# JohannesErnst/WeaSAL

Measured on AMD Instinct MI355X. Metric: points/sec fwd+bwd KPFCNN on DALES spheres; achieved HBM GB/s on KPConv gather, higher is better.
Workload: dtype f32; 1 GPU; DALES_PseudoLabel KP-FCNN, in_radius=10m, 50k pts/sphere, batch=8, fp32, step = GPU pyramid + fwd + loss + bwd + SGD; contrast_loss term included (trainer_PseudoLabel.py:204-208); pyramid of the next batch overlapped on a second stream; parallelism=dp1, dist_world_size=1, allreduce_bytes=0

## Files before the change

### weasal_amd/csrc/blocks.hip

```cpp
#include <vector>

#include "ws_common.h"

extern "C" int ws_block_gates = 1;
extern "C" int ws_block_gather_residual = 1;
extern "C" int64_t ws_block_group_rows = (int64_t)1 << 62;
extern "C" int ws_block_fused_infer = 1;
extern "C" int ws_block_pool_order = 1;
extern "C" int ws_block_packed_k4 = 1;

namespace {

struct Arena {
    char* base;
    int64_t cap, off;
    Arena(void* b, int64_t c) : base((char*)b), cap(c), off(0) {}
    template <typename T> T* take(int64_t count)
    {
        off = (off + 255) & ~(int64_t)255;
        T* p = base ? reinterpret_cast<T*>(base + off) : nullptr;
        off += count * (int64_t)sizeof(T);
        return p;
    }
    bool fits() const { return off <= cap; }
// ... 32 lines not shown
               int act, float slope, float* y, float* tr, void* tmp, int64_t tmp_bytes, hipStream_t st)
{
    if (l.in_place())
        return ws_gemm_xb_epilogue_strided(x, m, l.k, ldx, l.w, 1, l.ldw, l.n, bias, residual, ldr, act, slope, y, l.n, tmp, tmp_bytes, st);
    transpose_small_kernel<<<(unsigned)ws_ceil_div((int64_t)l.k * l.n, 256), 256, 0, st>>>(l.w, l.n, l.k, l.ldw, tr);
    return ws_gemm_xb_epilogue_strided(x, m, l.k, ldx, tr, l.n, 1, l.n, bias, residual, ldr, act, slope, y, l.n, tmp, tmp_bytes, st);
}

#define WS_TRY(call)            \
    do {                        \
        int rc__ = (call);      \
        if (rc__) return rc__;  \
    } while (0)

inline bool grouped_rows(int64_t rows) { return ws_block_group_rows > 0 && rows > 0 && rows < ws_block_group_rows; }

inline ws_xb_problem xb_problem(const float* x, int64_t m, int k, int64_t ldx, const float* b, int64_t brs, int64_t bcs, int n,
                                const float* bias, const float* residual, int64_t ldr, int act, float slope, const float* gate_y,
                                int64_t ldg, float gate_slope, float* y, int64_t ldy, void* scratch, int64_t scratch_bytes)
{
    ws_xb_problem q{};
    q.x = x; q.m = m; q.k = k; q.ldx = ldx; q.b = b; q.b_row_stride = brs; q.b_col_stride = bcs; q.n = n;
    q.bias = bias; q.residual = residual; q.ldr = ldr; q.act = act; q.slope = slope;
    q.gate_y = gate_y; q.ldg = ldg; q.gate_slope = gate_slope;
    q.y = y; q.ldy = ldy; q.scratch = scratch; q.scratch_bytes = scratch_bytes;
    return q;
}

struct Leaves {
    bool on;
// ... 52 lines not shown
{
    int64_t t = ws_gemm_xb_scratch_bytes(d->nq, d->k * d->conv_in, d->conv_out);
    if (d->w1) t = max3(t, ws_gemm_xb_scratch_bytes(d->ns, d->in_dim, d->conv_in), 0);
    if (d->w2) t = max3(t, ws_gemm_xb_scratch_bytes(d->nq, d->conv_out, d->out_dim), d->ws ? ws_gemm_xb_scratch_bytes(d->nq, d->in_dim, d->out_dim) : 0);
    return t;
}

int kpblock_fwd(const ws_kpblock* d, Arena& ar, hipStream_t st, bool run)
{
    const int64_t nq = d->nq, ns = d->ns;
    const Lin l1{d->w1, d->conv_in, d->in_dim, d->in_dim}, l2{d->w2, d->out_dim, d->conv_out, d->conv_out},
        lsc{d->ws, d->out_dim, d->in_dim, d->in_dim};
    float* tr1 = d->w1 ? ar.take<float>(l1.tr_floats()) : nullptr;
    float* tr2 = d->w2 ? ar.take<float>(l2.tr_floats()) : nullptr;
    float* trs = d->ws ? ar.take<float>(lsc.tr_floats()) : nullptr;
    float* sc = (d->w2 && d->ws) ? ar.take<float>(nq * d->out_dim) : nullptr;
    const int64_t tmp_bytes = kpblock_tmp_fwd(d);
    void* tmp = ar.take<char>(tmp_bytes > 16 ? tmp_bytes : 16);
    const bool pair_in = grouped_rows(nq) && d->w1 && d->w2 && d->ws && !d->strided && l1.in_place() && lsc.in_place();
    const int64_t sc_bytes = pair_in ? ws_gemm_xb_scratch_bytes(nq, d->in_dim, d->out_dim) : 0;
    void* tmp_sc = pair_in ? (void*)ar.take<char>(sc_bytes > 16 ? sc_bytes : 16) : nullptr;
    if (!run) return WS_OK;
    if (nq == 0) return WS_OK;
    const float* x1 = d->feat;
    if (pair_in) {
        const ws_xb_problem q[2] = {
            xb_problem(d->feat, ns, l1.k, d->in_dim, l1.w, 1, l1.ldw, l1.n, d->b1, nullptr, 0, 1, d->slope, nullptr, 0, 0.0f, d->x1, l1.n,
                       tmp, tmp_bytes),
            xb_problem(d->feat, nq, lsc.k, d->in_dim, lsc.w, 1, lsc.ldw, lsc.n, d->bs, nullptr, 0, 0, 0.0f, nullptr, 0, 0.0f, sc, lsc.n,
                       tmp_sc, sc_bytes)};
        WS_TRY(ws_priv_gemm_xb_group(q, 2, st));
        x1 = d->x1;
    } else if (d->w1) {
        WS_TRY(linear_fwd(l1, d->feat, ns, d->in_dim, d->b1, nullptr, 0, 1, d->slope, d->x1, tr1, tmp, tmp_bytes, st));
        x1 = d->x1;
    }
    TimerRec rec{};
    if (d->timed) {
        WS_HIP(hipEventCreate(&rec.a));
        WS_HIP(hipEventCreate(&rec.b));
        rec.nq = nq; rec.h = d->h; rec.ci = d->conv_in;
        WS_HIP(hipEventRecord(rec.a, st));
    }
    float* x2 = d->w2 ? d->x2 : d->out;
    const bool one_launch = d->infer && d->k == 15 && d->conv_in == 32 && d->conv_out == 32 && !d->rows_sorted && ((uintptr_t)x1 & 15u) == 0 &&
// ... 5 lines not shown
    } else {
        WS_REQUIRE(d->wf, "wf buffer missing");
        WS_TRY(ws_kpconv_gather_fwd_ex(d->q_pts, nq, d->s_pts, ns, d->inds, d->h, x1, d->conv_in, d->kernel_points, d->k, nullptr,
                                       nullptr, d->extent, WS_INFLUENCE_LINEAR, WS_AGGREGATION_SUM, d->order_q, d->wf, nullptr, 0,
                                       d->rows_sorted, st));
        if (d->timed) WS_HIP(hipEventRecord(rec.b, st));
        WS_TRY(ws_gemm_xb_epilogue_strided(d->wf, nq, d->k * d->conv_in, (int64_t)d->k * d->conv_in, d->wk, d->conv_out, 1, d->conv_out,
                                           d->bk, nullptr, 0, 1, d->slope, x2, d->conv_out, tmp, tmp_bytes, st));
    }
    if (d->timed) {
        WS_HIP(hipEventCreate(&rec.c));
        WS_HIP(hipEventRecord(rec.c, st));
        timer_recs().push_back(rec);
    }
    if (!d->w2) return WS_OK;
    const float* sc_in = d->feat;
    if (d->strided) {
        if (arg_bytes(d))
            WS_TRY(ws_priv_max_pool_fwd_u8(d->feat, ns, d->in_dim, d->inds, nq, d->h, d->pooled, reinterpret_cast<uint8_t*>(d->arg),
                                           ws_block_pool_order ? d->order_q : nullptr, st));
        else
            WS_TRY(ws_max_pool_fwd(d->feat, ns, d->in_dim, d->inds, nq, d->h, d->pooled, d->arg, st));
        sc_in = d->pooled;
    }
    const float* res = sc_in;
    int64_t ldr = d->in_dim;
    if (d->ws) {
        if (!pair_in) WS_TRY(linear_fwd(lsc, sc_in, nq, d->in_dim, d->bs, nullptr, 0, 0, 0.0f, sc, trs, tmp, tmp_bytes, st));
        res = sc;
        ldr = d->out_dim;
    }
    return linear_fwd(l2, x2, nq, d->conv_out, d->b2, res, ldr, 1, d->slope, d->out, tr2, tmp, tmp_bytes, st);
}

int kpblock_bwd(const ws_kpblock* d, Arena& ar, hipStream_t st, bool run)
{
    const int64_t nq = d->nq, ns = d->ns;
    const int kc = d->k * d->conv_in;
    const bool need_dx1 = d->dfeat != nullptr || d->w1 != nullptr;
    const bool want_sc = d->w2 && d->dfeat;
    float* dz = d->w2 ? ar.take<float>(nq * d->out_dim) : nullptr;
    float* g2 = ar.take<float>(nq * d->conv_out);
    float* dwf = need_dx1 ? ar.take<float>(nq * (int64_t)kc) : nullptr;
    float* dx1 = (need_dx1 && d->w1) ? ar.take<float>(ns * d->conv_in) : nullptr;
    float* dscin = (want_sc && d->ws) ? ar.take<float>(nq * d->in_dim) : nullptr;
    float* dfsc = (want_sc && d->strided) ? ar.take<float>(ns * d->in_dim) : nullptr;
    const Lin lk{d->wk, kc, d->conv_out, d->conv_out};
    float* trk = need_dx1 ? ar.take<float>(lk.tr_floats()) : nullptr;
    int64_t tmp_bytes = max3(ws_act_bwd_colsum_scratch_bytes(nq, d->out_dim > d->conv_out ? d->out_dim : d->conv_out),
                             ws_act_bwd_colsum_scratch_bytes(ns, d->conv_in), ws_gemm_xty_scratch_bytes(nq, kc, d->conv_out));
    if (d->w2) tmp_bytes = max3(tmp_bytes, ws_gemm_xty_scratch_bytes(nq, d->out_dim, d->conv_out),
                                d->ws ? ws_gemm_xty_scratch_bytes(nq, d->out_dim, d->in_dim) : 0);
    if (d->w1) tmp_bytes = max3(tmp_bytes, ws_gemm_xty_scratch_bytes(ns, d->conv_in, d->in_dim), 0);
    tmp_bytes = max3(tmp_bytes, ws_gemm_xb_scratch_bytes(nq, d->conv_out, kc), ws_gemm_xb_scratch_bytes(nq, d->out_dim, d->conv_out));
    tmp_bytes = max3(tmp_bytes, ws_gemm_xb_scratch_bytes(nq, d->out_dim, d->in_dim), ws_gemm_xb_scratch_bytes(ns, d->conv_in, d->in_dim));
    void* tmp = ar.take<char>(tmp_bytes > 16 ? tmp_bytes : 16);
    const bool grp = grouped_rows(nq > ns ? nq : ns) && nq > 0 && ns > 0;
    const int64_t b_dwk = ws_gemm_xty_scratch_bytes(nq, kc, d->conv_out);
    const int64_t b_dw2 = d->w2 ? ws_gemm_xty_scratch_bytes(nq, d->out_dim, d->conv_out) : 0;
    const int64_t b_dws = (d->w2 && d->ws) ? ws_gemm_xty_scratch_bytes(nq, d->out_dim, d->in_dim) : 0;
    const int64_t b_dw1 = d->w1 ? ws_gemm_xty_scratch_bytes(ns, d->conv_in, d->in_dim) : 0;
    const int64_t b_g2 = d->w2 ? ws_gemm_xb_scratch_bytes(nq, d->out_dim, d->conv_out) : 0;
    auto own = [&](int64_t bytes) -> void* { return grp ? (void*)ar.take<char>(bytes > 16 ? bytes : 16) : tmp; };
    void* t_dwk = own(b_dwk);
    void* t_dw2 = d->w2 ? own(b_dw2) : tmp;
    void* t_dws = (d->w2 && d->ws) ? own(b_dws) : tmp;
    void* t_dw1 = d->w1 ? own(b_dw1) : tmp;
    void* t_g2 = d->w2 ? own(b_g2) : tmp;
    if (!run) return WS_OK;
    WS_REQUIRE(d->dout && d->dwk, "NULL gradient buffer");
// ... 20 lines not shown
    const float* yconv = d->out;
    WS_REQUIRE(!(d->gate_dfeat && d->dfeat_add && !(d->strided && want_sc)),
               "gate_dfeat with dfeat_add needs the strided shortcut (the sum has to be complete before the gate)");
    if (d->w2) {
        if (d->dout_pregated) {
            if (d->db2) WS_TRY(ws_act_bwd_colsum(d->dout, nq, d->out_dim, d->out_dim, nullptr, 0, 0.0f, nullptr, 0, d->db2, tmp, st));
            dz = const_cast<float*>(d->dout);
        } else
        WS_TRY(ws_act_bwd_colsum(d->dout, nq, d->out_dim, d->out_dim, d->out, d->out_dim, d->slope, dz, d->out_dim, d->db2, tmp, st));
        WS_TRY(leaves.add(dz, nq, d->out_dim, d->out_dim, d->x2, d->conv_out, d->conv_out, d->dw2, 0, t_dw2, b_dw2));
        if (d->ws) {
            const float* sc_in = d->strided ? d->pooled : d->feat;
            WS_TRY(leaves.add(dz, nq, d->out_dim, d->out_dim, sc_in, d->in_dim, d->in_dim, d->dws, 0, t_dws, b_dws));
        }
        gated2 = !d->dbk && ws_block_gates;
        const bool pair_dz = grp && want_sc && d->ws;
        if (pair_dz) {
            const ws_xb_problem q[2] = {
                xb_problem(dz, nq, d->out_dim, d->out_dim, d->ws, d->in_dim, 1, d->in_dim, nullptr, nullptr, 0, 0, 0.0f, nullptr, 0, 0.0f,
                           dscin, d->in_dim, tmp, tmp_bytes),
                xb_problem(dz, nq, d->out_dim, d->out_dim, d->w2, d->conv_out, 1, d->conv_out, nullptr, nullptr, 0, 0, 0.0f,
                           gated2 ? d->x2 : nullptr, d->conv_out, d->slope, g2, d->conv_out, t_g2, b_g2)};
            WS_TRY(ws_priv_gemm_xb_group(q, 2, st));
        }
        if (want_sc) {
            const float* dsc = dz;
            if (d->ws) {
                if (!pair_dz)
                    WS_TRY(ws_gemm_xb_epilogue_strided(dz, nq, d->out_dim, d->out_dim, d->ws, d->in_dim, 1, d->in_dim, nullptr, nullptr, 0,
                                                       0, 0.0f, dscin, d->in_dim, tmp, tmp_bytes, st));
                dsc = dscin;
            }
            if (d->strided) {
                WS_REQUIRE(d->t_offsets && d->t_pairs, "strided block backward needs the transposed table");
                if (arg_bytes(d))
                {
                    WS_TRY(ws_priv_max_pool_bwd_u8(dsc, reinterpret_cast<const uint8_t*>(d->arg), nq, d->h, d->in_dim, d->t_offsets,
                                                   d->t_pairs, ns, dfsc, ws_block_pool_order ? d->order_s : nullptr, d->dfeat_add, st));
                    added = d->dfeat_add != nullptr;
                }
// ... 34 lines not shown
        WS_REQUIRE(d->key_last && d->grid_overflow && nq == ns, "grid backward needs key_last / overflow and a self-query layer");
        WS_TRY(ws_kpconv_gather_bwd_x_grid_gated(d->s_pts, ns, d->grid_blob, d->grid_nb, d->grid_cells, d->key_last, d->grid_radius, dwf,
                                                 d->conv_in, d->kernel_points, d->k, nullptr, nullptr, d->extent, WS_INFLUENCE_LINEAR,
                                                 WS_AGGREGATION_SUM, d->order_s, gate1, d->slope, d->inds, d->h, dx1_out,
                                                 d->grid_overflow, st));
    } else {
        WS_REQUIRE(d->t_offsets && d->t_pairs, "KPConv backward needs the search grid or the transposed table");
        WS_TRY((ws_block_packed_k4 ? ws_kpconv_gather_bwd_x_packed : ws_kpconv_gather_bwd_x_gated)(
            d->q_pts, nq, d->s_pts, ns, d->inds, d->h, d->t_offsets, d->t_pairs, dwf, d->conv_in, d->kernel_points, d->k, nullptr, nullptr,
            d->extent, WS_INFLUENCE_LINEAR, WS_AGGREGATION_SUM, d->order_s, gate1, d->slope, dx1_out, st));
    }
    if (d->w1) {
        if (!gate1)
            WS_TRY(ws_act_bwd_colsum(dx1, ns, d->conv_in, d->conv_in, d->x1, d->conv_in, d->slope, dx1, d->conv_in, d->db1, tmp, st));
        WS_TRY(leaves.add(dx1, ns, d->conv_in, d->conv_in, d->feat, d->in_dim, d->in_dim, d->dw1, 0, t_dw1, b_dw1));
        if (d->dfeat)
            WS_TRY(ws_gemm_xb_gated_strided(dx1, ns, d->conv_in, d->conv_in, d->w1, d->in_dim, 1, d->in_dim, nullptr, sc_res, d->in_dim,
                                            0, 0.0f, d->gate_dfeat ? d->feat : nullptr, d->in_dim, d->slope, nullptr, 0, 0.0f, d->dfeat,
                                            d->in_dim, tmp, tmp_bytes, st));
    } else if (d->dfeat && sc_res) {
        WS_REQUIRE(!d->gate_dfeat, "gate_dfeat: a block without unary1 has no shortcut to add after the gate");
        const int64_t n4 = ns * d->in_dim / 4;
        add_rows_kernel<<<ws_grid(n4, 256), 256, 0, st>>>(d->dfeat, sc_res, n4);
        WS_LAUNCH_CHECK();
    }
    if (d->dfeat && d->dfeat_add && !added) {
        WS_REQUIRE(d->in_dim % 4 == 0, "dfeat_add needs in_dim %% 4 == 0");
        const int64_t n4 = ns * d->in_dim / 4;
        add_rows_kernel<<<ws_grid(n4, 256), 256, 0, st>>>(d->dfeat, d->dfeat_add, n4);
        WS_LAUNCH_CHECK();
    }
// ... 202 lines not shown
```

### weasal_amd/csrc/gemm.hip

```cpp
#include "gemm_launch.h"

using namespace gemm;

extern "C" {
int ws_gemm_shallow = 1;
int ws_gemm_staged = 1;
}

namespace {

int64_t colsum_chunk(int64_t m)
{
    int64_t c = ws_ceil_div(m, 768);
    return c < 16 ? 16 : c;
}

bool al16(const void* p) { return (reinterpret_cast<uintptr_t>(p) & 15u) == 0; }

bool reduce_partials_wide(const void* partial, int64_t elems, int chunks, const void* out, int n, int64_t ldo)
{
    return elems >= 65536 && chunks <= 64 && elems % 4 == 0 && al16(partial) && al16(out) && (ldo <= n || (n % 4 == 0 && ldo % 4 == 0));
}

int64_t xty_chunk(int64_t m, int k, int n)
// ... 106 lines not shown
    }
    if (rc != WS_OK) return rc;
    WS_LAUNCH_CHECK();
    return WS_OK;
}

int xb_run(const ws_xb_problem& q, void* stream)
{
    int rc = xb_validate(q, -1);
    if (rc != WS_OK || q.m == 0) return rc;
    XbPlan p;
    rc = xb_plan(q, p);
    return rc != WS_OK ? rc : xb_launch(q, p, (hipStream_t)stream);
}

ws_xb_problem xb_problem(const float* x, int64_t m, int32_t k, int64_t ldx, const float* b, int32_t n, float* y, int64_t ldy,
                         void* scratch = nullptr, int64_t scratch_bytes = 0)
{
    ws_xb_problem q{};
    q.x = x; q.m = m; q.k = k; q.ldx = ldx;
    q.b = b; q.b_row_stride = -1; q.b_col_stride = 1; q.n = n;
    q.y = y; q.ldy = ldy;
    q.scratch = scratch; q.scratch_bytes = scratch_bytes;
    return q;
}
void xb_epilogue(ws_xb_problem& q, const float* bias, const float* residual, int64_t ldr, int32_t act, float slope)
{
    q.bias = bias; q.residual = residual; q.ldr = ldr; q.act = act; q.slope = slope;
}
void xb_strides(ws_xb_problem& q, int64_t b_row_stride, int64_t b_col_stride)
// ... 229 lines not shown
            if (rc != WS_OK) return rc;
            continue;
        }
        if (xb2_pair(p.nt, p.wn) < 0) return xb2_no_instantiation(p);
        bucket[xb2_pair(p.nt, p.wn)].push_back(i);
    }
    for (const IdList& ids : bucket) {
        const int rc = for_each_launch(ids, [&](const int* id, int cnt) {
            return cnt == 1 ? xb_launch(q[id[0]], plan[id[0]], st) : launch_xb2_group(q, plan, id, cnt, st);
        });
        if (rc != WS_OK) return rc;
    }
    return WS_OK;
}

int64_t ws_act_bwd_colsum_scratch_bytes(int64_t m, int32_t n)
{
    return ws_ceil_div(m > 0 ? m : 1, colsum_chunk(m)) * (int64_t)n * (int64_t)sizeof(float);
}

static ColsumPlan colsum_plan(const void* dy, int64_t m, int32_t n, int64_t lddy, const void* y, int64_t ldy, const void* dz,
                              int64_t lddz, float* colsum, void* scratch)
{
    ColsumPlan p{};
    p.chunk = colsum_chunk(m);
    p.chunks = (int)ws_ceil_div(m, p.chunk);
    p.partial = colsum ? (p.chunks == 1 ? colsum : (float*)scratch) : nullptr;
    p.reduce = colsum && p.chunks > 1;
    const bool vec = n % 4 == 0 && al16(dy) && lddy % 4 == 0 && (!y || (al16(y) && ldy % 4 == 0 && al16(dz) && lddz % 4 == 0));
    p.v = vec ? 4 : 1;
// ... 117 lines not shown
    if (rc == WS_OK) rc = xb_plan(q, p);
    if (rc != WS_OK) return rc;
    if (p.kind == XB_NONE)
        snprintf(out, (size_t)cap, "none (m == 0)");
    else if (p.kind == XB_XB2)
        snprintf(out, (size_t)cap, "gemm_xb2_kernel<NT=%d, WN=%d> b=%s epilogue=%s splits=%d csplit=%d%s", p.nt, p.wn,
                 xb_brs(q) == 1 ? "transposed" : "rows", p.staged ? "staged" : "lanes", p.splits, p.csplit,
                 p.splits > 1 ? " + splitk_epilogue_kernel" : "");
    else if (p.kind == XB_SHALLOW)
        snprintf(out, (size_t)cap, "gemm_xb_shallow_kernel rows=%d", p.rows);
    else
        snprintf(out, (size_t)cap, "gemm_xb_kernel<NT=%d, BKX=32> vecx=%d vecb=%d", p.nt, p.vecx, p.vecb);
    return WS_OK;
}

int ws_gemm_xty_variant(const void* x, int64_t m, int32_t k, int64_t ldx, const void* y, int32_t n, int64_t ldy, float* out_m,
                        int64_t ldo, void* scratch, int32_t rows_bf16, char* out, int32_t cap)
{
    WS_REQUIRE(out && cap > 0, "bad argument");
    WS_REQUIRE(!rows_bf16 || ldo == 0, "the bf16 reduction has no pitched form");
    const ws_xty_problem q{(const float*)x, m, k, ldx, (const float*)y, n, ldy, out_m, ldo, scratch, 0};
    XtyPlan p;
    int rc = xty_validate(q, -1);
    if (rc == WS_OK) rc = xty_plan(q, rows_bf16 != 0, p);
    if (rc != WS_OK) return rc;
    const char* form = p.pitched ? "pitched" : "flat";
    if (m == 0)
        snprintf(out, (size_t)cap, "memset (m == 0) out=%s", form);
    else if (!p.lds)
        snprintf(out, (size_t)cap, "gemm_xty2_kernel<KT=%d, NT=%d, WK=%d, WN=%d, TI=%s> chunk=%lld chunks=%d reduce=%s out=%s", p.kt, p.nt,
// ... 24 lines not shown
```

### weasal_amd/csrc/gemm_launch.h

```cpp
#pragma once
#include "ws_dispatch.h"

namespace gemm {

constexpr int BM = 128;
constexpr int BK = 32;
constexpr int GROUP_MAX = 8;

inline int64_t xb_brs(const ws_xb_problem& q) { return q.b_row_stride < 0 ? q.n : q.b_row_stride; }

enum { XB_NONE = 0, XB_XB2 = 1, XB_SHALLOW = 2, XB_GENERIC = 3 };
struct XbPlan {
    int kind;
    int nt, wn;
    dim3 grid;
    int splits, csplit;
    int staged;
    int vecx, vecb;
    int rows;
    size_t lds;
};

constexpr int XB2_PAIRS[][2] = {{1, 1}, {2, 1}, {4, 1}, {1, 2}, {2, 2}};
constexpr int XB2_NPAIRS = 5;
constexpr int xb2_pair(int nt, int wn)
{
    for (int i = 0; i < XB2_NPAIRS; ++i)
        if (XB2_PAIRS[i][0] == nt && XB2_PAIRS[i][1] == wn) return i;
    return -1;
}
inline int xb2_no_instantiation(const XbPlan& p) { return ws_no_instantiation("gemm_xb2_kernel<NT=%d, WN=%d>", p.nt, p.wn); }

struct XtyPlan {
    int bf16;
    int lds;
    int kt, nt, wk, wn;
    int vecx, vecy;
    int64_t chunk;
    int chunks;
    float* partial;
    int reduce;
    bool pitched;
    dim3 grid;
};

struct ColsumPlan {
    int v;
    int64_t chunk;
    int chunks;
    float* partial;
    int reduce;
    dim3 grid;
};

#pragma GCC visibility push(hidden)
int launch_xb2(const ws_xb_problem& q, const XbPlan& p, hipStream_t st);
void launch_splitk_epilogue(const ws_xb_problem& q, const XbPlan& p, hipStream_t st);
void launch_xb_shallow(const ws_xb_problem& q, const XbPlan& p, hipStream_t st);
int launch_xb_generic(const ws_xb_problem& q, const XbPlan& p, hipStream_t st);
int launch_xb2_group(const ws_xb_problem* q, const XbPlan* plan, const int* ids, int cnt, hipStream_t st);
int launch_xty2(const ws_xty_problem& q, const XtyPlan& p, hipStream_t st);
int launch_xty_lds(const ws_xty_problem& q, const XtyPlan& p, hipStream_t st);
void launch_reduce_partials(bool wide, const float* partial, int64_t elems, int chunks, float* out, hipStream_t st, int n = 0,
                            int64_t ldo = 0);
int launch_xty2_group(const ws_xty_problem* q, const XtyPlan* plan, const int* ids, int cnt, hipStream_t st);
void launch_reduce_group(const ws_xty_problem* q, const XtyPlan* plan, const int* ids, int cnt, hipStream_t st);
int launch_act_bwd_colsum(const ColsumPlan& p, const float* dy, int64_t m, int32_t n, int64_t lddy, const float* y, int64_t ldy,
                          float slope, float* dz, int64_t lddz, const WsDrop& drop, hipStream_t st);
#pragma GCC visibility pop

}
```

### weasal_amd/csrc/gemm_xb.hip

```cpp
#include "gemm_device.h"

namespace {

template <int NT, int BKX>
__global__ __launch_bounds__(256) void gemm_xb_kernel(const float* __restrict__ x, int64_t m, int k, int64_t ldx,
                                                       const float* __restrict__ b, int n, int64_t ldb,
                                                       float* __restrict__ y, int64_t ldy, int vecx, int vecb,
                                                       const float* __restrict__ bias, const float* __restrict__ residual,
                                                       int64_t ldr, int act, float slope, const XbGate gate)
{
    constexpr int BN = 32 * NT;
    __shared__ float Xs[BM][BKX + 1];
    __shared__ __attribute__((aligned(16))) float Bs[BKX][BN];
    const int t = threadIdx.x;
    const int wave = __builtin_amdgcn_readfirstlane(t >> 6);
    const int lane = t & 63;
    const int64_t m0 = (int64_t)blockIdx.x * BM;
    const int n0 = blockIdx.y * BN;
    constexpr int XCOLS4 = BKX / 4;
    constexpr int XROWS = 256 / XCOLS4;
    constexpr int XPT = BM / XROWS;
    const int xr = t / XCOLS4, xc = (t % XCOLS4) * 4;
    constexpr int BPT = (BKX * BN / 4 + 255) / 256;
    f32x16 acc[NT];
// ... 316 lines not shown
    int k, n, ldb, bcs, act, csplit, staged; float slope;
    unsigned gx, gy;
};
struct Xb2Group { GroupIndex gi; Xb2Problem p[GROUP_MAX]; };
static_assert(sizeof(Xb2Group) < 4096, "the group travels in the kernel arguments");

template <int NT, int WN>
__global__ __launch_bounds__(256) __attribute__((amdgpu_waves_per_eu(3))) void gemm_xb2_group_kernel(const Xb2Group g)
{
    unsigned l;
    const Xb2Problem& p = g.p[group_find(g.gi, l)];
    const unsigned gx = p.gx, gy = p.gy;
    const unsigned bx = l % gx, q = l / gx;
    gemm_xb2_body<NT, WN>(bx, q % gy, q / gy, p.x, p.m, p.k, p.ldx, p.b, p.n, p.ldb, p.bcs, p.y, p.ldy, p.bias, p.residual, p.ldr,
                          p.act, p.slope, p.csplit, p.partial, p.gate, p.staged);
}

__global__ __launch_bounds__(256) void gemm_xb_shallow_kernel(const float* __restrict__ x, int64_t m, int k, int64_t ldx,
                                                               const float* __restrict__ b, int n, float* __restrict__ y, int64_t ldy,
                                                               const float* __restrict__ bias, const float* __restrict__ residual,
                                                               int64_t ldr, int act, float slope, const XbGate gate, int rows_per_wg)
{
    extern __shared__ __attribute__((aligned(16))) float shallow_lds[];
    const int kp = (k + 3) & ~3;
    float* bs = shallow_lds;
    float* xs = shallow_lds + kp * n;
    const int t = threadIdx.x;
    for (int e = t; e < kp * n / 4; e += 256)
        reinterpret_cast<float4*>(bs)[e] = e < k * n / 4 ? reinterpret_cast<const float4*>(b)[e] : make_float4(0.f, 0.f, 0.f, 0.f);
    const int64_t r0 = (int64_t)blockIdx.x * rows_per_wg;
// ... 130 lines not shown
int launch_xb2(const ws_xb_problem& q, const XbPlan& p, hipStream_t st)
{
    const XbGate gate = xb_problem_gate(q);
    float* part = p.splits > 1 ? (float*)q.scratch : nullptr;
    bool pruned = false;
    const bool called = dispatch([&](auto nt, auto wn) {
        if constexpr (xb2_pair(nt.value, wn.value) >= 0)
            gemm_xb2_kernel<nt.value, wn.value><<<p.grid, 256, 0, st>>>(q.x, q.m, q.k, q.ldx, q.b, q.n, (int)xb_brs(q), (int)q.b_col_stride, q.y,
                                                                        q.ldy, q.bias, q.residual, q.ldr, q.act, q.slope, p.csplit, part, gate,
                                                                        p.staged);
        else pruned = true;
    }, Pick<1, 2, 4>{p.nt}, Pick<1, 2>{p.wn});
    return called && !pruned ? WS_OK : xb2_no_instantiation(p);
}

void launch_splitk_epilogue(const ws_xb_problem& q, const XbPlan& p, hipStream_t st)
{
    splitk_epilogue_kernel<<<ws_grid(q.m * (q.n / 4), 256), 256, 0, st>>>((const float*)q.scratch, p.splits, q.m, q.n, q.y, q.ldy, q.bias,
                                                                          q.residual, q.ldr, q.act, q.slope, xb_problem_gate(q));
}

void launch_xb_shallow(const ws_xb_problem& q, const XbPlan& p, hipStream_t st)
{
    gemm_xb_shallow_kernel<<<p.grid, 256, p.lds, st>>>(q.x, q.m, q.k, q.ldx, q.b, q.n, q.y, q.ldy, q.bias, q.residual, q.ldr, q.act, q.slope,
                                                       xb_problem_gate(q), p.rows);
}

int launch_xb_generic(const ws_xb_problem& q, const XbPlan& p, hipStream_t st)
{
    const XbGate gate = xb_problem_gate(q);
// ... 48 lines not shown
```

### weasal_amd/csrc/ws_common.h

```cpp
#pragma once
#include <hip/hip_runtime.h>
#include <stdint.h>
#include <stdio.h>
#include <stdarg.h>
#include "../../include/weasal_hip.h"

#define WS_WAVE 64

char* ws_errbuf();
inline int ws_fail(int code, const char* fmt, ...)
{
    va_list ap;
    va_start(ap, fmt);
    vsnprintf(ws_errbuf(), 512, fmt, ap);
    va_end(ap);
    return code;
}

#define WS_HIP(call)                                                                     \
    do {                                                                                 \
        hipError_t e__ = (call);                                                         \
        if (e__ != hipSuccess)                                                           \
            return ws_fail(WS_ERR_HIP, "%s failed: %s (%s:%d)", #call, hipGetErrorString(e__), \
                           __FILE__, __LINE__);                                          \
// ... 36 lines not shown
    const float* gate_y; int64_t ldg; float gate_slope;
    const uint8_t* mask; int64_t ldm; float mask_scale;
    float drop_p; uint64_t drop_seed;
    float* y; int64_t ldy;
    void* scratch; int64_t scratch_bytes;
};
struct ws_xty_problem {
    const float* x; int64_t m; int32_t k; int64_t ldx;
    const float* y; int32_t n; int64_t ldy;
    float* out; int64_t ldo;
    void* scratch; int64_t scratch_bytes;
};
extern "C" int ws_priv_gemm_xb_group(const ws_xb_problem* p, int32_t count, void* stream);
extern "C" int ws_priv_gemm_xty_group(const ws_xty_problem* p, int32_t count, void* stream);

static inline int ws_grid(int64_t items, int per_block, int max_blocks = 256 * 16)
{
    int64_t b = ws_ceil_div(items, per_block);
    if (b < 1) b = 1;
    if (b > max_blocks) b = max_blocks;
    if (b > 8) b = (b + 7) / 8 * 8;
    return (int)b;
}

#ifdef __HIPCC__
__device__ __forceinline__ int ws_lane() { return threadIdx.x & 63; }
__device__ __forceinline__ float ws_readlane_f(float v, int lane)
{
    return __int_as_float(__builtin_amdgcn_readlane(__float_as_int(v), lane));
}
// ... 58 lines not shown
```

### weasal_amd/fused.py

```python
import ctypes as C
import os
import weakref

import torch

from . import _lib, ops
from ._lib import check, current_stream

FUSED_BLOCKS = os.environ.get("WEASAL_FUSED_BLOCKS", "1") != "0"
FUSED_INFER = os.environ.get("WEASAL_FUSED_INFER", "1") != "0"
_timed = False


_timed_min_rows = 0


def set_timed(on, min_rows=0):
    global _timed, _timed_min_rows
    _timed = bool(on)
    _timed_min_rows = int(min_rows)


_vp, _i32, _i64, _f32 = C.c_void_p, C.c_int32, C.c_int64, C.c_float

# ... 8 lines not shown

_GATES_SET = False


def _bind():
    global _GATES_SET
    lib = _lib.lib()
    if not _GATES_SET:
        C.c_int.in_dll(lib, "ws_block_gates").value = 0 if os.environ.get("WEASAL_BLOCK_GATES", "1") == "0" else 1
        C.c_int.in_dll(lib, "ws_block_fused_infer").value = 1 if FUSED_INFER else 0
        C.c_int.in_dll(lib, "ws_block_gather_residual").value = 0 if os.environ.get("WEASAL_BLOCK_GATHER_RESIDUAL", "1") == "0" else 1
        C.c_int.in_dll(lib, "ws_block_pool_order").value = 0 if os.environ.get("WEASAL_POOL_ORDER", "1") == "0" else 1
        C.c_int.in_dll(lib, "ws_block_packed_k4").value = 0 if os.environ.get("WEASAL_BLOCK_PACKED_K4", "1") == "0" else 1
        if "WEASAL_BLOCK_GROUP_ROWS" in os.environ:
            C.c_int64.in_dll(lib, "ws_block_group_rows").value = int(os.environ["WEASAL_BLOCK_GROUP_ROWS"])
        _GATES_SET = True
    return lib


def timer_records(layer=False):
    lib = _bind()
    out = []
    nq, h, ci, ms, ml = _i64(), _i32(), _i32(), _f32(), _f32()
    for i in range(lib.ws_timer_count()):
        check(lib.ws_timer_read(i, C.byref(nq), C.byref(h), C.byref(ci), C.byref(ms)))
        if layer:
            check(lib.ws_timer_read_layer(i, C.byref(ml)))
            out.append((nq.value, h.value, ci.value, ms.value, ml.value))
        else:
            out.append((nq.value, h.value, ci.value, ms.value))
# ... 374 lines not shown
```

Baseline: 33.14 million points/s.

## Fold shortcut GEMM into second unary GEMM via dual-chain MFMA kernel

Adds a dual-chain GEMM kernel that accumulates two X·B products, each with its own bias, into the same register tile and applies one shared epilogue. In the residual block forward pass it computes the shortcut linear and the second unary linear together, and in the backward pass it computes the shortcut gradient and the dfeat product together. This avoids materialising the shortcut output and dscin buffers and saves a separate launch plus the residual read. The fold is only used for blocks with at least 32768 query rows whose shapes map to compatible tile configurations. The cost is a bigger kernel with two sequential K loops per tile.

```diff
diff --git a/weasal_amd/csrc/blocks.hip b/weasal_amd/csrc/blocks.hip
--- a/weasal_amd/csrc/blocks.hip
+++ b/weasal_amd/csrc/blocks.hip
@@ -8,6 +8,7 @@
 extern "C" int ws_block_fused_infer = 1;
 extern "C" int ws_block_pool_order = 1;
 extern "C" int ws_block_packed_k4 = 1;
+extern "C" int64_t ws_block_fold_rows = 32768;
 
 namespace {
 
@@ -70,6 +71,8 @@
     } while (0)
 
 inline bool grouped_rows(int64_t rows) { return ws_block_group_rows > 0 && rows > 0 && rows < ws_block_group_rows; }
+inline bool fold_rows(int64_t rows) { return rows > 0 && rows >= ws_block_fold_rows; }
+template <typename T> inline T* arena_standin() { return reinterpret_cast<T*>((uintptr_t)256); }
 
 inline ws_xb_problem xb_problem(const float* x, int64_t m, int k, int64_t ldx, const float* b, int64_t brs, int64_t bcs, int n,
                                 const float* bias, const float* residual, int64_t ldr, int act, float slope, const float* gate_y,
@@ -152,10 +155,23 @@
     float* tr1 = d->w1 ? ar.take<float>(l1.tr_floats()) : nullptr;
     float* tr2 = d->w2 ? ar.take<float>(l2.tr_floats()) : nullptr;
     float* trs = d->ws ? ar.take<float>(lsc.tr_floats()) : nullptr;
-    float* sc = (d->w2 && d->ws) ? ar.take<float>(nq * d->out_dim) : nullptr;
     const int64_t tmp_bytes = kpblock_tmp_fwd(d);
+    auto unary2 = [&](void* scratch) {
+        return xb_problem(d->x2, nq, l2.k, d->conv_out, l2.w, 1, l2.ldw, l2.n, d->b2, nullptr, 0, 1, d->slope, nullptr, 0, 0.0f, d->out, l2.n,
+                          scratch, tmp_bytes);
+    };
+    auto shortcut = [&](float* y, void* scratch, int64_t bytes) {
+        return xb_problem(d->feat, nq, lsc.k, d->in_dim, lsc.w, 1, lsc.ldw, lsc.n, d->bs, nullptr, 0, 0, 0.0f, nullptr, 0, 0.0f, y, lsc.n,
+                          scratch, bytes);
+    };
+    bool fold = fold_rows(nq) && d->w1 && d->w2 && d->ws && !d->strided && l2.in_place() && lsc.in_place();
+    if (fold) {
+        const ws_xb_problem a = unary2(arena_standin<void>()), r = shortcut(arena_standin<float>(), arena_standin<void>(), tmp_bytes);
+        fold = ws_priv_gemm_xb_dual_folds(&a, &r) != 0;
+    }
+    float* sc = (d->w2 && d->ws && !fold) ? ar.take<float>(nq * d->out_dim) : nullptr;
     void* tmp = ar.take<char>(tmp_bytes > 16 ? tmp_bytes : 16);
-    const bool pair_in = grouped_rows(nq) && d->w1 && d->w2 && d->ws && !d->strided && l1.in_place() && lsc.in_place();
+    const bool pair_in = !fold && grouped_rows(nq) && d->w1 && d->w2 && d->ws && !d->strided && l1.in_place() && lsc.in_place();
     const int64_t sc_bytes = pair_in ? ws_gemm_xb_scratch_bytes(nq, d->in_dim, d->out_dim) : 0;
     void* tmp_sc = pair_in ? (void*)ar.take<char>(sc_bytes > 16 ? sc_bytes : 16) : nullptr;
     if (!run) return WS_OK;
@@ -165,8 +181,7 @@
         const ws_xb_problem q[2] = {
             xb_problem(d->feat, ns, l1.k, d->in_dim, l1.w, 1, l1.ldw, l1.n, d->b1, nullptr, 0, 1, d->slope, nullptr, 0, 0.0f, d->x1, l1.n,
                        tmp, tmp_bytes),
-            xb_problem(d->feat, nq, lsc.k, d->in_dim, lsc.w, 1, lsc.ldw, lsc.n, d->bs, nullptr, 0, 0, 0.0f, nullptr, 0, 0.0f, sc, lsc.n,
-                       tmp_sc, sc_bytes)};
+            shortcut(sc, tmp_sc, sc_bytes)};
         WS_TRY(ws_priv_gemm_xb_group(q, 2, st));
         x1 = d->x1;
     } else if (d->w1) {
@@ -202,6 +217,12 @@
         timer_recs().push_back(rec);
     }
     if (!d->w2) return WS_OK;
+    if (fold) {
+        const ws_xb_problem a = unary2(tmp), r = shortcut(nullptr, tmp, tmp_bytes);
+        const int rc = ws_priv_gemm_xb_dual(&a, &r, st);
+        WS_REQUIRE(rc != WS_XB_DUAL_DECLINED, "the folded shortcut was planned but declined at the launch");
+        return rc;
+    }
     const float* sc_in = d->feat;
     if (d->strided) {
         if (arg_bytes(d))
@@ -227,14 +248,6 @@
     const int kc = d->k * d->conv_in;
     const bool need_dx1 = d->dfeat != nullptr || d->w1 != nullptr;
     const bool want_sc = d->w2 && d->dfeat;
-    float* dz = d->w2 ? ar.take<float>(nq * d->out_dim) : nullptr;
-    float* g2 = ar.take<float>(nq * d->conv_out);
-    float* dwf = need_dx1 ? ar.take<float>(nq * (int64_t)kc) : nullptr;
-    float* dx1 = (need_dx1 && d->w1) ? ar.take<float>(ns * d->conv_in) : nullptr;
-    float* dscin = (want_sc && d->ws) ? ar.take<float>(nq * d->in_dim) : nullptr;
-    float* dfsc = (want_sc && d->strided) ? ar.take<float>(ns * d->in_dim) : nullptr;
-    const Lin lk{d->wk, kc, d->conv_out, d->conv_out};
-    float* trk = need_dx1 ? ar.take<float>(lk.tr_floats()) : nullptr;
     int64_t tmp_bytes = max3(ws_act_bwd_colsum_scratch_bytes(nq, d->out_dim > d->conv_out ? d->out_dim : d->conv_out),
                              ws_act_bwd_colsum_scratch_bytes(ns, d->conv_in), ws_gemm_xty_scratch_bytes(nq, kc, d->conv_out));
     if (d->w2) tmp_bytes = max3(tmp_bytes, ws_gemm_xty_scratch_bytes(nq, d->out_dim, d->conv_out),
@@ -242,6 +255,28 @@
     if (d->w1) tmp_bytes = max3(tmp_bytes, ws_gemm_xty_scratch_bytes(ns, d->conv_in, d->in_dim), 0);
     tmp_bytes = max3(tmp_bytes, ws_gemm_xb_scratch_bytes(nq, d->conv_out, kc), ws_gemm_xb_scratch_bytes(nq, d->out_dim, d->conv_out));
     tmp_bytes = max3(tmp_bytes, ws_gemm_xb_scratch_bytes(nq, d->out_dim, d->in_dim), ws_gemm_xb_scratch_bytes(ns, d->conv_in, d->in_dim));
+    auto dfeat_product = [&](const float* dx1_, void* scratch) {
+        return xb_problem(dx1_, ns, d->conv_in, d->conv_in, d->w1, d->in_dim, 1, d->in_dim, nullptr, nullptr, 0, 0, 0.0f,
+                          d->gate_dfeat ? d->feat : nullptr, d->in_dim, d->slope, d->dfeat, d->in_dim, scratch, tmp_bytes);
+    };
+    auto dsc_product = [&](const float* dz_, float* y, void* scratch) {
+        return xb_problem(dz_, nq, d->out_dim, d->out_dim, d->ws, d->in_dim, 1, d->in_dim, nullptr, nullptr, 0, 0, 0.0f, nullptr, 0, 0.0f, y,
+                          d->in_dim, scratch, tmp_bytes);
+    };
+    bool fold = fold_rows(nq) && want_sc && d->ws && d->w1 && !d->strided;
+    if (fold) {
+        const ws_xb_problem a = dfeat_product(arena_standin<float>(), arena_standin<void>()),
+                            r = dsc_product(d->dout_pregated ? d->dout : arena_standin<float>(), arena_standin<float>(), arena_standin<void>());
+        fold = ws_priv_gemm_xb_dual_folds(&a, &r) != 0;
+    }
+    float* dz = d->w2 ? ar.take<float>(nq * d->out_dim) : nullptr;
+    float* g2 = ar.take<float>(nq * d->conv_out);
+    float* dwf = need_dx1 ? ar.take<float>(nq * (int64_t)kc) : nullptr;
+    float* dx1 = (need_dx1 && d->w1) ? ar.take<float>(ns * d->conv_in) : nullptr;
+    float* dscin = (want_sc && d->ws && !fold) ? ar.take<float>(nq * d->in_dim) : nullptr;
+    float* dfsc = (want_sc && d->strided) ? ar.take<float>(ns * d->in_dim) : nullptr;
+    const Lin lk{d->wk, kc, d->conv_out, d->conv_out};
+    float* trk = need_dx1 ? ar.take<float>(lk.tr_floats()) : nullptr;
     void* tmp = ar.take<char>(tmp_bytes > 16 ? tmp_bytes : 16);
     const bool grp = grouped_rows(nq > ns ? nq : ns) && nq > 0 && ns > 0;
     const int64_t b_dwk = ws_gemm_xty_scratch_bytes(nq, kc, d->conv_out);
@@ -292,16 +327,15 @@
             WS_TRY(leaves.add(dz, nq, d->out_dim, d->out_dim, sc_in, d->in_dim, d->in_dim, d->dws, 0, t_dws, b_dws));
         }
         gated2 = !d->dbk && ws_block_gates;
-        const bool pair_dz = grp && want_sc && d->ws;
+        const bool pair_dz = grp && want_sc && d->ws && !fold;
         if (pair_dz) {
             const ws_xb_problem q[2] = {
-                xb_problem(dz, nq, d->out_dim, d->out_dim, d->ws, d->in_dim, 1, d->in_dim, nullptr, nullptr, 0, 0, 0.0f, nullptr, 0, 0.0f,
-                           dscin, d->in_dim, tmp, tmp_bytes),
+                dsc_product(dz, dscin, tmp),
                 xb_problem(dz, nq, d->out_dim, d->out_dim, d->w2, d->conv_out, 1, d->conv_out, nullptr, nullptr, 0, 0, 0.0f,
                            gated2 ? d->x2 : nullptr, d->conv_out, d->slope, g2, d->conv_out, t_g2, b_g2)};
             WS_TRY(ws_priv_gemm_xb_group(q, 2, st));
         }
-        if (want_sc) {
+        if (want_sc && !fold) {
             const float* dsc = dz;
             if (d->ws) {
                 if (!pair_dz)
@@ -366,7 +400,12 @@
         if (!gate1)
             WS_TRY(ws_act_bwd_colsum(dx1, ns, d->conv_in, d->conv_in, d->x1, d->conv_in, d->slope, dx1, d->conv_in, d->db1, tmp, st));
         WS_TRY(leaves.add(dx1, ns, d->conv_in, d->conv_in, d->feat, d->in_dim, d->in_dim, d->dw1, 0, t_dw1, b_dw1));
-        if (d->dfeat)
+        if (fold) {
+            const ws_xb_problem a = dfeat_product(dx1, tmp), r = dsc_product(dz, nullptr, tmp);
+            const int rc = ws_priv_gemm_xb_dual(&a, &r, st);
+            WS_REQUIRE(rc != WS_XB_DUAL_DECLINED, "the folded shortcut gradient was planned but declined at the launch");
+            WS_TRY(rc);
+        } else if (d->dfeat)
             WS_TRY(ws_gemm_xb_gated_strided(dx1, ns, d->conv_in, d->conv_in, d->w1, d->in_dim, 1, d->in_dim, nullptr, sc_res, d->in_dim,
                                             0, 0.0f, d->gate_dfeat ? d->feat : nullptr, d->in_dim, d->slope, nullptr, 0, 0.0f, d->dfeat,
                                             d->in_dim, tmp, tmp_bytes, st));
diff --git a/weasal_amd/csrc/gemm.hip b/weasal_amd/csrc/gemm.hip
--- a/weasal_amd/csrc/gemm.hip
+++ b/weasal_amd/csrc/gemm.hip
@@ -144,6 +144,31 @@
     return rc != WS_OK ? rc : xb_launch(q, p, (hipStream_t)stream);
 }
 
+int xb_dual_plan(const ws_xb_problem& a, const ws_xb_problem& r_in, XbPlan& p, const char*& why)
+{
+    p = XbPlan{};
+    why = "";
+    ws_xb_problem r = r_in;
+    r.y = a.y; r.ldy = a.ldy;
+    int rc = xb_validate(a, 0);
+    if (rc == WS_OK) rc = xb_validate(r, 1);
+    if (rc != WS_OK) return rc;
+    if (a.m != r.m || a.n != r.n) { why = "m or n differ"; return WS_OK; }
+    if (a.m == 0) { why = "m == 0"; return WS_OK; }
+    if (a.residual || a.res_rows) { why = "the first product has a residual of its own"; return WS_OK; }
+    if (r.residual || r.res_rows || r.gate_y || r.mask || r.drop_p > 0.0f || r.act) { why = "the second product has an epilogue beyond its bias"; return WS_OK; }
+    XbPlan pa, pr;
+    rc = xb_plan(a, pa);
+    if (rc == WS_OK) rc = xb_plan(r, pr);
+    if (rc != WS_OK) return rc;
+    if (pa.kind != XB_XB2 || pr.kind != XB_XB2) { why = "a product does not take gemm_xb2_kernel"; return WS_OK; }
+    if (pa.splits != 1 || pr.splits != 1) { why = "a product is split"; return WS_OK; }
+    if (pa.nt != pr.nt || pa.wn != pr.wn) { why = "the products take different <NT, WN>"; return WS_OK; }
+    if (!xb2_dual_pair(pa.nt, pa.wn)) { why = "no two-chain kernel for this <NT, WN>"; return WS_OK; }
+    p = pa;
+    return WS_OK;
+}
+
 ws_xb_problem xb_problem(const float* x, int64_t m, int32_t k, int64_t ldx, const float* b, int32_t n, float* y, int64_t ldy,
                          void* scratch = nullptr, int64_t scratch_bytes = 0)
 {
@@ -403,6 +428,27 @@
     return WS_OK;
 }
 
+int ws_priv_gemm_xb_dual(const ws_xb_problem* first, const ws_xb_problem* second, void* stream)
+{
+    WS_REQUIRE(first && second, "NULL problem");
+    XbPlan p;
+    const char* why;
+    int rc = xb_dual_plan(*first, *second, p, why);
+    if (rc != WS_OK) return rc;
+    if (p.kind == XB_NONE) return WS_XB_DUAL_DECLINED;
+    rc = launch_xb2_dual(*first, *second, p, (hipStream_t)stream);
+    if (rc != WS_OK) return rc;
+    WS_LAUNCH_CHECK();
+    return WS_OK;
+}
+
+int ws_priv_gemm_xb_dual_folds(const ws_xb_problem* first, const ws_xb_problem* second)
+{
+    XbPlan p;
+    const char* why;
+    return first && second && xb_dual_plan(*first, *second, p, why) == WS_OK && p.kind == XB_XB2;
+}
+
 int64_t ws_act_bwd_colsum_scratch_bytes(int64_t m, int32_t n)
 {
     return ws_ceil_div(m > 0 ? m : 1, colsum_chunk(m)) * (int64_t)n * (int64_t)sizeof(float);
@@ -550,6 +596,21 @@
     return WS_OK;
 }
 
+int ws_priv_gemm_xb_dual_variant(const ws_xb_problem* first, const ws_xb_problem* second, char* out, int32_t cap)
+{
+    WS_REQUIRE(first && second && out && cap > 0, "bad argument");
+    XbPlan p;
+    const char* why;
+    const int rc = xb_dual_plan(*first, *second, p, why);
+    if (rc != WS_OK) return rc;
+    if (p.kind == XB_NONE)
+        snprintf(out, (size_t)cap, "none (%s)", why);
+    else
+        snprintf(out, (size_t)cap, "gemm_xb2_dual_kernel<NT=%d, WN=%d> b1=%s b2=%s epilogue=%s", p.nt, p.wn,
+                 xb_brs(*first) == 1 ? "transposed" : "rows", xb_brs(*second) == 1 ? "transposed" : "rows", p.staged ? "staged" : "lanes");
+    return WS_OK;
+}
+
 int ws_gemm_xty_variant(const void* x, int64_t m, int32_t k, int64_t ldx, const void* y, int32_t n, int64_t ldy, float* out_m,
                         int64_t ldo, void* scratch, int32_t rows_bf16, char* out, int32_t cap)
 {
diff --git a/weasal_amd/csrc/gemm_launch.h b/weasal_amd/csrc/gemm_launch.h
--- a/weasal_amd/csrc/gemm_launch.h
+++ b/weasal_amd/csrc/gemm_launch.h
@@ -30,6 +30,7 @@
     return -1;
 }
 inline int xb2_no_instantiation(const XbPlan& p) { return ws_no_instantiation("gemm_xb2_kernel<NT=%d, WN=%d>", p.nt, p.wn); }
+constexpr bool xb2_dual_pair(int nt, int wn) { return nt <= 2 && xb2_pair(nt, wn) >= 0; }
 
 struct XtyPlan {
     int bf16;
@@ -59,6 +60,7 @@
 void launch_xb_shallow(const ws_xb_problem& q, const XbPlan& p, hipStream_t st);
 int launch_xb_generic(const ws_xb_problem& q, const XbPlan& p, hipStream_t st);
 int launch_xb2_group(const ws_xb_problem* q, const XbPlan* plan, const int* ids, int cnt, hipStream_t st);
+int launch_xb2_dual(const ws_xb_problem& a, const ws_xb_problem& r, const XbPlan& p, hipStream_t st);
 int launch_xty2(const ws_xty_problem& q, const XtyPlan& p, hipStream_t st);
 int launch_xty_lds(const ws_xty_problem& q, const XtyPlan& p, hipStream_t st);
 void launch_reduce_partials(bool wide, const float* partial, int64_t elems, int chunks, float* out, hipStream_t st, int n = 0,
diff --git a/weasal_amd/csrc/gemm_xb.hip b/weasal_amd/csrc/gemm_xb.hip
--- a/weasal_amd/csrc/gemm_xb.hip
+++ b/weasal_amd/csrc/gemm_xb.hip
@@ -354,6 +354,159 @@
     const unsigned bx = l % gx, q = l / gx;
     gemm_xb2_body<NT, WN>(bx, q % gy, q / gy, p.x, p.m, p.k, p.ldx, p.b, p.n, p.ldb, p.bcs, p.y, p.ldy, p.bias, p.residual, p.ldr,
                           p.act, p.slope, p.csplit, p.partial, p.gate, p.staged);
+}
+
+struct Xb2Chain { const float* x; int64_t ldx; const float* b; const float* bias; int k, ldb, bcs; };
+
+template <int NT, int WN>
+__device__ __forceinline__ void xb2_dual_chain(f32x16 (&acc)[NT], float* __restrict__ Ws, const Xb2Chain& c, int64_t brow0, int64_t brows,
+                                               int n0, int n, int t, int wm, int wn, int idx, int h)
+{
+    constexpr int CT = NT * WN;
+    constexpr int BN = 32 * CT;
+    constexpr int KC = 32;
+    constexpr int WBUF = CT * 1024;
+    const int k = c.k, ldb = c.ldb, bcs = c.bcs;
+    const auto wsrd = __builtin_amdgcn_make_buffer_rsrc(const_cast<float*>(c.b), 0,
+                                                        (int)(((int64_t)(k - 1) * ldb + (int64_t)(n - 1) * bcs + 1) * 4), 0x00020000);
+    const auto xsrd = __builtin_amdgcn_make_buffer_rsrc(const_cast<float*>(c.x + brow0 * c.ldx), 0,
+                                                        (int)(((brows - 1) * c.ldx + k) * 4), 0x00020000);
+    int woff[CT];
+    int wlds[CT];
+    const bool wtr = ldb == 1;
+#pragma unroll
+    for (int i = 0; i < CT; ++i) {
+        const int g = t + 256 * i;
+        const int cc = wtr ? g / 8 : g % BN, q = wtr ? g % 8 : g / BN;
+        int col = n0 + cc;
+        col = col < n ? col : n - 1;
+        woff[i] = (4 * q * ldb + col * bcs) * 4;
+        wlds[i] = ((((cc >> 5) * 4 + (q >> 1)) * 2 + (q & 1)) * 32 + (cc & 31)) * 4;
+    }
+    float4 wv[CT];
+    auto load_w = [&](int chunk) {
+        const int so = chunk * KC * ldb * 4;
+        if (wtr) {
+#pragma unroll
+            for (int i = 0; i < CT; ++i) {
+                const u32x4 v = __builtin_amdgcn_raw_buffer_load_b128(wsrd, woff[i], so, 0);
+                wv[i] = make_float4(__uint_as_float(v.x), __uint_as_float(v.y), __uint_as_float(v.z), __uint_as_float(v.w));
+            }
+            return;
+        }
+#pragma unroll
+        for (int i = 0; i < CT; ++i) {
+            wv[i].x = __uint_as_float(__builtin_amdgcn_raw_buffer_load_b32(wsrd, woff[i], so, 0));
+            wv[i].y = __uint_as_float(__builtin_amdgcn_raw_buffer_load_b32(wsrd, woff[i], so + ldb * 4, 0));
+            wv[i].z = __uint_as_float(__builtin_amdgcn_raw_buffer_load_b32(wsrd, woff[i], so + ldb * 8, 0));
+            wv[i].w = __uint_as_float(__builtin_amdgcn_raw_buffer_load_b32(wsrd, woff[i], so + ldb * 12, 0));
+        }
+    };
+    auto store_w = [&](int buf) {
+#pragma unroll
+        for (int i = 0; i < CT; ++i) *reinterpret_cast<float4*>(&Ws[buf * WBUF + wlds[i]]) = wv[i];
+    };
+    const int xoff = (int)((wm * 32 + idx) * c.ldx + 4 * h) * 4;
+    float4 xn[4], xc[4];
+    auto load_x = [&](int chunk) {
+#pragma unroll
+        for (int j = 0; j < 4; ++j) {
+            const u32x4 v = __builtin_amdgcn_raw_buffer_load_b128(xsrd, xoff + 32 * j, chunk * (KC * 4), 0);
+            xn[j] = make_float4(__uint_as_float(v.x), __uint_as_float(v.y), __uint_as_float(v.z), __uint_as_float(v.w));
+        }
+    };
+
+    const int cend = k / KC, last = cend - 1;
+    load_w(0);
+    load_x(0);
+    {
+        float4 w0[CT];
+#pragma unroll
+        for (int i = 0; i < CT; ++i) w0[i] = wv[i];
+        load_w(last < 1 ? last : 1);
+#pragma unroll
+        for (int i = 0; i < CT; ++i) *reinterpret_cast<float4*>(&Ws[wlds[i]]) = w0[i];
+    }
+    __syncthreads();
+    for (int cc = 0; cc < cend; ++cc) {
+#pragma unroll
+        for (int j = 0; j < 4; ++j) xc[j] = xn[j];
+        store_w((cc + 1) & 1);
+        load_x(cc + 1 < last ? cc + 1 : last);
+        load_w(cc + 2 < last ? cc + 2 : last);
+        const float* wb = &Ws[(cc & 1) * WBUF + wn * (NT * 1024) + (h * 32 + idx) * 4];
+#pragma unroll
+        for (int j = 0; j < 4; ++j) {
+            __builtin_amdgcn_sched_barrier(0);
+#pragma unroll
+            for (int i = 0; i < NT; ++i) {
+                const float4 a4 = *reinterpret_cast<const float4*>(wb + (i * 4 + j) * 256);
+                acc[i] = __builtin_amdgcn_mfma_f32_32x32x2f32(a4.x, xc[j].x, acc[i], 0, 0, 0);
+                acc[i] = __builtin_amdgcn_mfma_f32_32x32x2f32(a4.y, xc[j].y, acc[i], 0, 0, 0);
+                acc[i] = __builtin_amdgcn_mfma_f32_32x32x2f32(a4.z, xc[j].z, acc[i], 0, 0, 0);
+                acc[i] = __builtin_amdgcn_mfma_f32_32x32x2f32(a4.w, xc[j].w, acc[i], 0, 0, 0);
+            }
+        }
+        __syncthreads();
+    }
+}
+
+template <int NT, int WN>
+__global__ __launch_bounds__(256) __attribute__((amdgpu_waves_per_eu(WN == 1 ? 4 : 3))) void gemm_xb2_dual_kernel(
+    const Xb2Chain c1, const Xb2Chain c2, int64_t m, int n, float* __restrict__ y, int64_t ldy, int act, float slope, const XbGate gate,
+    int staged)
+{
+    constexpr int WM = 4 / WN;
+    constexpr int CT = NT * WN;
+    constexpr int WBUF = CT * 1024;
+    constexpr int WS_FLOATS = 2 * WBUF > 4 * XB_STAGE_FLOATS ? 2 * WBUF : 4 * XB_STAGE_FLOATS;
+    __shared__ __attribute__((aligned(16))) float Ws[WS_FLOATS];
+    const int t = threadIdx.x;
+    const int wave = __builtin_amdgcn_readfirstlane(t >> 6);
+    const int wm = wave / WN, wn = wave % WN;
+    const int lane = t & 63;
+    const int idx = lane & 31, h = lane >> 5;
+    const int64_t brow0 = (int64_t)blockIdx.x * (32 * WM);
+    const int64_t brows = m - brow0 < 32 * WM ? m - brow0 : 32 * WM;
+    const int n0 = blockIdx.y * (32 * CT);
+    const int n0w = n0 + wn * (32 * NT);
+
+    f32x16 acc[NT], r[NT];
+#pragma unroll
+    for (int i = 0; i < NT; ++i)
+#pragma unroll
+        for (int e = 0; e < 16; ++e) acc[i][e] = 0.0f;
+    xb2_dual_chain<NT, WN>(acc, Ws, c2, brow0, brows, n0, n, t, wm, wn, idx, h);
+#pragma unroll
+    for (int i = 0; i < NT; ++i)
+#pragma unroll
+        for (int g = 0; g < 4; ++g) {
+            const int col = n0w + 32 * i + 8 * g + 4 * h;
+            float4 bq = make_float4(0.f, 0.f, 0.f, 0.f);
+            if (c2.bias) bq = *reinterpret_cast<const float4*>(c2.bias + (col < n ? col : n - 4));
+            if (staged) {
+                r[i][4 * g + 0] = (acc[i][4 * g + 0] + 0.0f) + bq.x; r[i][4 * g + 1] = (acc[i][4 * g + 1] + 0.0f) + bq.y;
+                r[i][4 * g + 2] = (acc[i][4 * g + 2] + 0.0f) + bq.z; r[i][4 * g + 3] = (acc[i][4 * g + 3] + 0.0f) + bq.w;
+            } else if (c2.bias) {
+                r[i][4 * g + 0] = acc[i][4 * g + 0] + bq.x; r[i][4 * g + 1] = acc[i][4 * g + 1] + bq.y;
+                r[i][4 * g + 2] = acc[i][4 * g + 2] + bq.z; r[i][4 * g + 3] = acc[i][4 * g + 3] + bq.w;
+            } else {
+                r[i][4 * g + 0] = acc[i][4 * g + 0]; r[i][4 * g + 1] = acc[i][4 * g + 1];
+                r[i][4 * g + 2] = acc[i][4 * g + 2]; r[i][4 * g + 3] = acc[i][4 * g + 3];
+            }
+        }
+#pragma unroll
+    for (int i = 0; i < NT; ++i)
+#pragma unroll
+        for (int e = 0; e < 16; ++e) acc[i][e] = 0.0f;
+    xb2_dual_chain<NT, WN>(acc, Ws, c1, brow0, brows, n0, n, t, wm, wn, idx, h);
+#pragma unroll
+    for (int i = 0; i < NT; ++i) acc[i] = acc[i] + r[i];
+    if (staged)
+        xb_rows_epilogue_staged<NT>(acc, brow0 + wm * 32, m, n0w, n, lane, y, ldy, c1.bias, nullptr, 0, act, slope, gate,
+                                    &Ws[wave * XB_STAGE_FLOATS]);
+    else
+        xb_rows_epilogue<NT>(acc, brow0 + wm * 32 + idx, m, n0w, n, h, y, ldy, c1.bias, nullptr, 0, act, slope, gate);
 }
 
 __global__ __launch_bounds__(256) void gemm_xb_shallow_kernel(const float* __restrict__ x, int64_t m, int k, int64_t ldx,
@@ -514,6 +667,21 @@
     return called && !pruned ? WS_OK : xb2_no_instantiation(p);
 }
 
+int launch_xb2_dual(const ws_xb_problem& a, const ws_xb_problem& r, const XbPlan& p, hipStream_t st)
+{
+    const Xb2Chain c1{a.x, a.ldx, a.b, a.bias, a.k, (int)xb_brs(a), (int)a.b_col_stride};
+    const Xb2Chain c2{r.x, r.ldx, r.b, r.bias, r.k, (int)xb_brs(r), (int)r.b_col_stride};
+    const XbGate gate = xb_problem_gate(a);
+    bool pruned = false;
+    const bool called = dispatch([&](auto nt, auto wn) {
+        if constexpr (xb2_dual_pair(nt.value, wn.value))
+            gemm_xb2_dual_kernel<nt.value, wn.value><<<dim3(p.grid.x, p.grid.y), 256, 0, st>>>(c1, c2, a.m, a.n, a.y, a.ldy, a.act, a.slope, gate,
+                                                                                                p.staged);
+        else pruned = true;
+    }, Pick<1, 2, 4>{p.nt}, Pick<1, 2>{p.wn});
+    return called && !pruned ? WS_OK : ws_no_instantiation("gemm_xb2_dual_kernel<NT=%d, WN=%d>", p.nt, p.wn);
+}
+
 void launch_splitk_epilogue(const ws_xb_problem& q, const XbPlan& p, hipStream_t st)
 {
     splitk_epilogue_kernel<<<ws_grid(q.m * (q.n / 4), 256), 256, 0, st>>>((const float*)q.scratch, p.splits, q.m, q.n, q.y, q.ldy, q.bias,
diff --git a/weasal_amd/csrc/ws_common.h b/weasal_amd/csrc/ws_common.h
--- a/weasal_amd/csrc/ws_common.h
+++ b/weasal_amd/csrc/ws_common.h
@@ -74,6 +74,11 @@
 extern "C" int ws_priv_gemm_xb_group(const ws_xb_problem* p, int32_t count, void* stream);
 extern "C" int ws_priv_gemm_xty_group(const ws_xty_problem* p, int32_t count, void* stream);
 
+#define WS_XB_DUAL_DECLINED (-1)
+extern "C" int ws_priv_gemm_xb_dual(const ws_xb_problem* first, const ws_xb_problem* second, void* stream);
+extern "C" int ws_priv_gemm_xb_dual_folds(const ws_xb_problem* first, const ws_xb_problem* second);
+extern "C" int ws_priv_gemm_xb_dual_variant(const ws_xb_problem* first, const ws_xb_problem* second, char* out, int32_t cap);
+
 static inline int ws_grid(int64_t items, int per_block, int max_blocks = 256 * 16)
 {
     int64_t b = ws_ceil_div(items, per_block);
diff --git a/weasal_amd/fused.py b/weasal_amd/fused.py
--- a/weasal_amd/fused.py
+++ b/weasal_amd/fused.py
@@ -46,6 +46,8 @@
         C.c_int.in_dll(lib, "ws_block_packed_k4").value = 0 if os.environ.get("WEASAL_BLOCK_PACKED_K4", "1") == "0" else 1
         if "WEASAL_BLOCK_GROUP_ROWS" in os.environ:
             C.c_int64.in_dll(lib, "ws_block_group_rows").value = int(os.environ["WEASAL_BLOCK_GROUP_ROWS"])
+        if "WEASAL_BLOCK_FOLD_ROWS" in os.environ:
+            C.c_int64.in_dll(lib, "ws_block_fold_rows").value = int(os.environ["WEASAL_BLOCK_FOLD_ROWS"])
         _GATES_SET = True
     return lib
 
```

Result: no change. 33.09 million points/s (-0.2%).
